# noc-lab/sac-expert

Measured on NVIDIA B200. Metric: agent-updates/sec, higher is better.
Workload: dtype f32

## Files before the change

sac_expert_b200/csrc/mlp_ws.cuh:

```cuda
#pragma once
#include "tc_gemm.cuh"
#include "planes.cuh"

namespace saceo {

constexpr int WS_NEW = 16;
constexpr int WS_NEPI = WS_NEW * 32, WS_NT = WS_NEPI + 64;
constexpr int WS_NST = 3, WS_RING = WS_NST * WS_STAGE;
constexpr int WS_AUX = 49152;
constexpr int WS_PATCH1 = 32 * 32 * 4;
constexpr int WS_PATCH = WS_NEW * WS_PATCH1;
constexpr int WS_MAIN = WS_RING + WS_AUX + WS_PATCH;
constexpr int WS_BYTES = WS_MAIN + 1024 + 256;
constexpr int WS_RED = 40960;
constexpr int WS_MAXOUT = 36;
enum { WB_FULL = 0, WB_EMPTY = WS_NST, WB_XFULL = 2 * WS_NST, WB_XEMPTY, WB_D0, WB_D1, WB_AP , WB_D2 = WB_AP + 4 };

__device__ __forceinline__ void mbar_arrive(uint32_t bar) {
  asm volatile("mbarrier.arrive.shared::cta.b64 _, [%0];" ::"r"(bar) : "memory");
}
__device__ __forceinline__ void mbar_expect_tx(uint32_t bar, uint32_t bytes) {
  asm volatile("mbarrier.arrive.expect_tx.shared::cta.b64 _, [%0], %1;" ::"r"(bar), "r"(bytes) : "memory");
}
__device__ __forceinline__ void bulk_g2s(uint32_t dst, const void* src, uint32_t bytes, uint32_t bar) {
  asm volatile("cp.async.bulk.shared::cluster.global.mbarrier::complete_tx::bytes [%0], [%1], %2, [%3];"
               ::"r"(dst), "l"(src), "r"(bytes), "r"(bar) : "memory");
}
__device__ __forceinline__ void bulk_prefetch_l2(const void* src, uint32_t bytes) {
  asm volatile("cp.async.bulk.prefetch.L2.global [%0], %1;" ::"l"(src), "r"(bytes) : "memory");
}
__device__ __forceinline__ void epi_bar() { asm volatile("bar.sync 1, 512;" ::: "memory"); }
__device__ __forceinline__ uint64_t umma_desc_mn(uint32_t saddr, uint32_t lbo = 4096) {
  return (uint64_t)((saddr >> 4) & 0x3FFF) | ((uint64_t)(lbo >> 4) << 16) | ((uint64_t)(1024 >> 4) << 32) |
         ((uint64_t)1 << 46) | ((uint64_t)2 << 61);
}
constexpr uint32_t WS_IDESC_FWD = (1u << 4) | (1u << 16) | ((uint32_t)(256 >> 3) << 17) | ((uint32_t)(128 >> 4) << 24);
constexpr uint32_t WS_IDESC_BWD = (1u << 4) | ((uint32_t)(128 >> 3) << 17) | ((uint32_t)(128 >> 4) << 24);

__global__ void k_planes_build(const float* __restrict__ theta, long long stride, uint8_t* __restrict__ img, int K0, int nout) {
  const int n0 = (K0 + 31) / 32, N2 = ws_w2_rows(nout), rows = n0 * 32 + 256 + N2;
  const int item = blockIdx.x * blockDim.x + threadIdx.x;
  if (item >= rows * 32) return;
  const int row = item >> 5, c8 = item & 31;
  const float* th = theta + (long long)blockIdx.y * stride;
  uint8_t* net_img = img + (long long)blockIdx.y * ws_image_bytes(K0, nout);
  float x[8];
  if (row >= n0 * 32 + 256) {
    const int n = row - n0 * 32 - 256;
    const long long o = (long long)K0 * 256 + 256 + 65536 + 256 + (long long)(c8 * 8) * nout + n;
#pragma unroll
    for (int j = 0; j < 8; ++j) x[j] = n < nout ? th[o + (long long)j * nout] * WS_W2_SCALE : 0.f;
    uint4 hi, lo;
    split8<true>(x, hi, lo);
    uint8_t* dst = net_img + (long long)(n0 + 8) * WS_STAGE + ws_w2_off(N2, n, c8);
    *reinterpret_cast<uint4*>(dst) = hi;
    *reinterpret_cast<uint4*>(dst + N2 * 128) = lo;
    return;
  }
  if (row < n0 * 32) {
#pragma unroll
    for (int j = 0; j < 8; ++j) x[j] = row < K0 ? th[(long long)row * 256 + c8 * 8 + j] : 0.f;
  } else {
    const long long o = (long long)K0 * 256 + 256 + (long long)(row - n0 * 32) * 256 + c8 * 8;
#pragma unroll
    for (int j = 0; j < 8; ++j) x[j] = th[o + j];
  }
  uint4 hi, lo;
  split8<true>(x, hi, lo);
  uint8_t* dst = net_img + ws_image_off(row, c8);
  *reinterpret_cast<uint4*>(dst) = hi;
  *reinterpret_cast<uint4*>(dst + 16384) = lo;
}

__device__ __forceinline__ uint32_t ws_pa(uint32_t patch, int r, int c) {
  return patch + (uint32_t)(r * 128 + ((((c >> 2) ^ (r & 7)) << 4) | ((c & 3) << 2)));
}
__device__ __forceinline__ void ws_store_rows(uint32_t patch, const uint32_t (&v)[32], float* __restrict__ G, int rbase,
                                              int rows, int col, int lane, uint32_t cs = 0, int q = 0) {
#pragma unroll
  for (int j = 0; j < 8; ++j) sts128(ws_pa(patch, lane, 4 * j), make_uint4(v[4 * j], v[4 * j + 1], v[4 * j + 2], v[4 * j + 3]));
  __syncwarp();
  const int lr = lane >> 3, lc = (lane & 7) * 4;
  float4 sum = make_float4(0.f, 0.f, 0.f, 0.f);
#pragma unroll
  for (int rr = 0; rr < 32; rr += 4) {
    const int r = rr + lr, grow = rbase + r;
    if (grow < rows) {
      const float4 t4 = lds128(ws_pa(patch, r, lc));
      if (G) *reinterpret_cast<float4*>(G + (long long)grow * FW_H + col + lc) = t4;
      sum.x += t4.x; sum.y += t4.y; sum.z += t4.z; sum.w += t4.w;
    }
  }
  if (cs) {
#pragma unroll
    for (int o = 8; o <= 16; o <<= 1) {
      sum.x += __shfl_xor_sync(0xffffffffu, sum.x, o); sum.y += __shfl_xor_sync(0xffffffffu, sum.y, o);
      sum.z += __shfl_xor_sync(0xffffffffu, sum.z, o); sum.w += __shfl_xor_sync(0xffffffffu, sum.w, o);
    }
    if (lane < 8) sts128f(cs + (uint32_t)(q * FW_H + col + lc) * 4, sum.x, sum.y, sum.z, sum.w);
// ... 170 lines not shown
__device__ __forceinline__ void ws_split_store(uint32_t taddr, const uint32_t (&v)[32], float scale) {
#pragma unroll
  for (int h = 0; h < 2; ++h) {
    uint32_t hi[8], lo[8];
#pragma unroll
    for (int j = 0; j < 8; ++j) {
      const float x0 = __uint_as_float(v[16 * h + 2 * j]) * scale, x1 = __uint_as_float(v[16 * h + 2 * j + 1]) * scale;
      asm("cvt.rn.satfinite.f16x2.f32 %0, %1, %2;" : "=r"(hi[j]) : "f"(x1), "f"(x0));
      const float2 hf = __half22float2(*reinterpret_cast<const __half2*>(&hi[j]));
      asm("cvt.rn.satfinite.f16x2.f32 %0, %1, %2;" : "=r"(lo[j]) : "f"(x1 - hf.y), "f"(x0 - hf.x));
    }
    tmem_st8(taddr + 8 * h, hi);
    tmem_st8(taddr + 16 + 8 * h, lo);
  }
}
template <int ACT>
__device__ __forceinline__ void ws_mul_dact_p(uint32_t (&v)[32], uint32_t patch, int lane, float s) {
#pragma unroll
  for (int j = 0; j < 8; ++j) {
    const float4 h = lds128(ws_pa(patch, lane, 4 * j));
    v[4 * j] = __float_as_uint(__uint_as_float(v[4 * j]) * s * dact_from_out(ACT, h.x));
    v[4 * j + 1] = __float_as_uint(__uint_as_float(v[4 * j + 1]) * s * dact_from_out(ACT, h.y));
    v[4 * j + 2] = __float_as_uint(__uint_as_float(v[4 * j + 2]) * s * dact_from_out(ACT, h.z));
    v[4 * j + 3] = __float_as_uint(__uint_as_float(v[4 * j + 3]) * s * dact_from_out(ACT, h.w));
  }
  __syncwarp();
}
__device__ __forceinline__ void ws_mul_dact_p_rt(int act, uint32_t (&v)[32], uint32_t patch, int lane, float s) {
  if (act == ACT_RELU) ws_mul_dact_p<ACT_RELU>(v, patch, lane, s);
  else if (act == ACT_TANH) ws_mul_dact_p<ACT_TANH>(v, patch, lane, s);
  else ws_mul_dact_p<ACT_ELU>(v, patch, lane, s);
}
__device__ __forceinline__ void ws_rows_commit_p(uint32_t patch, int lane, const float4 (&t)[8]) {
  const int lr = lane >> 3, lc = (lane & 7) * 4;
#pragma unroll
  for (int i = 0; i < 8; ++i)
    sts128(ws_pa(patch, 4 * i + lr, lc), make_uint4(__float_as_uint(t[i].x), __float_as_uint(t[i].y), __float_as_uint(t[i].z), __float_as_uint(t[i].w)));
  __syncwarp();
}
__device__ __forceinline__ void ws_split_f16(const uint32_t (&v)[32], float scale, uint32_t (&hi)[16], uint32_t (&lo)[16]) {
#pragma unroll
  for (int j = 0; j < 16; ++j) {
    const float x0 = __uint_as_float(v[2 * j]) * scale, x1 = __uint_as_float(v[2 * j + 1]) * scale;
    asm("cvt.rn.satfinite.f16x2.f32 %0, %1, %2;" : "=r"(hi[j]) : "f"(x1), "f"(x0));
    const float2 hf = __half22float2(*reinterpret_cast<const __half2*>(&hi[j]));
    asm("cvt.rn.satfinite.f16x2.f32 %0, %1, %2;" : "=r"(lo[j]) : "f"(x1 - hf.y), "f"(x0 - hf.x));
  }
}
template <int ACT>
__device__ __forceinline__ void ws_bias_act(uint32_t (&v)[32], uint32_t bias) {
#pragma unroll
  for (int j = 0; j < 8; ++j) {
    const float4 b = lds128(bias + j * 16);
    v[4 * j] = __float_as_uint(apply_act(ACT, __uint_as_float(v[4 * j]) + b.x));
    v[4 * j + 1] = __float_as_uint(apply_act(ACT, __uint_as_float(v[4 * j + 1]) + b.y));
    v[4 * j + 2] = __float_as_uint(apply_act(ACT, __uint_as_float(v[4 * j + 2]) + b.z));
    v[4 * j + 3] = __float_as_uint(apply_act(ACT, __uint_as_float(v[4 * j + 3]) + b.w));
  }
}
__device__ __forceinline__ void ws_bias_act_rt(int act, uint32_t (&v)[32], uint32_t bias) {
  if (act == ACT_RELU) ws_bias_act<ACT_RELU>(v, bias);
  else if (act == ACT_TANH) ws_bias_act<ACT_TANH>(v, bias);
  else ws_bias_act<ACT_ELU>(v, bias);
}
template <int ACT>
__device__ __forceinline__ void ws_mul_dact(uint32_t (&v)[32], const float (&aux)[32], float s) {
#pragma unroll
  for (int j = 0; j < 32; ++j) v[j] = __float_as_uint(__uint_as_float(v[j]) * s * dact_from_out(ACT, aux[j]));
}
__device__ __forceinline__ void ws_mul_dact_rt(int act, uint32_t (&v)[32], const float (&aux)[32], float s) {
  if (act == ACT_RELU) ws_mul_dact<ACT_RELU>(v, aux, s);
  else if (act == ACT_TANH) ws_mul_dact<ACT_TANH>(v, aux, s);
  else ws_mul_dact<ACT_ELU>(v, aux, s);
}
__device__ __forceinline__ float ws_row_scale(float bound) {
  if (!(bound > 0.f) || !(bound < 3.0e38f)) return 1.f;
  int e;
  frexpf(bound, &e);
  e = 10 - e;
  e = e > 120 ? 120 : (e < -120 ? -120 : e);
  return ldexpf(1.f, e);
}

struct FwdW {
  const float* X; int ldx; long long sXa, sXn;
  const float* theta; long long sTa, sTn;
  const uint8_t* planes; long long sPa, sPn;
  float* H1; float* H2; long long sHa, sHn;
  uint8_t* H1p; long long sQa, sQn;
  float* Out; int ldo; long long sOa, sOn;
  int rows, K0, nout, nnet, act0, act1;
  unsigned long long* dbg;
};
#define WS_STAMP(i) do { if (f.dbg && lane == 0) f.dbg[(size_t)(blockIdx.y * gridDim.x + blockIdx.x) * 16 + (i)] = gtime(); } while (0)

__global__ void __launch_bounds__(WS_NT, 1) k_mlp_fwd_ws(FwdW f) {
  extern __shared__ uint8_t smem_raw[];
  const uint32_t sb = (smem_u32(smem_raw) + 1023u) & ~1023u;
  const uint32_t ring = sb, aux = sb + WS_RING, patch_base = aux + WS_AUX, bars = sb + WS_MAIN, tslot = bars + 8 * 16;
  auto bar = [&](int i) { return bars + 8u * (uint32_t)i; };
  const int z = blockIdx.y, agent = z / f.nnet, net = z - agent * f.nnet;
  const int row0 = blockIdx.x * TC_BM;
  const int warp = threadIdx.x >> 5, lane = threadIdx.x & 31;
  const int n0 = (f.K0 + 31) >> 5, nk64 = (f.K0 + 63) >> 6;
  const int N2 = ws_w2_rows(f.nout);
  const uint32_t idesc_out = (1u << 4) | ((uint32_t)(N2 >> 3) << 17) | ((uint32_t)(128 >> 4) << 24);

  if (threadIdx.x == 0) {
    for (int s = 0; s < 2 * WS_NST; ++s) mbar_init(bar(s), 1);
    mbar_init(bar(WB_XFULL), WS_NEW); mbar_init(bar(WB_XEMPTY), 1);
    mbar_init(bar(WB_D0), 1); mbar_init(bar(WB_D1), 1); mbar_init(bar(WB_D2), 1);
    for (int g = 0; g < 4; ++g) mbar_init(bar(WB_AP + g), 8);
    asm volatile("fence.mbarrier_init.release.cluster;" ::: "memory");
  }
  if (warp == WS_NEW + 1) {
    asm volatile("tcgen05.alloc.cta_group::1.sync.aligned.shared::cta.b32 [%0], %1;" ::"r"(tslot), "n"(512) : "memory");
    asm volatile("tcgen05.relinquish_alloc_permit.cta_group::1.sync.aligned;" ::: "memory");
  }
  asm volatile("tcgen05.fence::before_thread_sync;" ::: "memory");
  __syncthreads();
  asm volatile("tcgen05.fence::after_thread_sync;" ::: "memory");
  const uint32_t tmem = lds_u32(tslot);
  const uint32_t tP = tmem, tQ = tmem + 256;

  if (warp == WS_NEW) {
    if (lane == 0) {
      const uint8_t* img = f.planes + agent * f.sPa + net * f.sPn;
      const int total = n0 + 8 + (N2 ? 2 : 0);
      const uint32_t w2_item = (uint32_t)N2 * 512;
      auto item_src = [&](int it) { return it < n0 + 8 ? img + (long long)it * WS_STAGE : img + (long long)(n0 + 8) * WS_STAGE + (it - n0 - 8) * w2_item; };
      for (int it = 0; it < total; ++it) {
        const int s = it % WS_NST;
        const uint32_t bytes = it < n0 + 8 ? (uint32_t)WS_STAGE : w2_item;
        mbar_wait(bar(WB_EMPTY + s), (uint32_t)(((it / WS_NST) & 1) ^ 1));
        mbar_expect_tx(bar(WB_FULL + s), bytes);
        bulk_g2s(ring + s * WS_STAGE, item_src(it), bytes, bar(WB_FULL + s));
        if (it == WS_NST - 1)
          for (int j = WS_NST; j < total; ++j) bulk_prefetch_l2(item_src(j), j < n0 + 8 ? (uint32_t)WS_STAGE : w2_item);
      }
      WS_STAMP(11);
    }
  } else if (warp == WS_NEW + 1) {
    if (lane == 0) {
      int it = 0;
      for (int sl = 0; sl < nk64; ++sl) {
        mbar_wait(bar(WB_XFULL), (uint32_t)(sl & 1));
        asm volatile("tcgen05.fence::after_thread_sync;" ::: "memory");
        for (int hh = 0; hh < 2 && sl * 2 + hh < n0; ++hh, ++it) {
          const int s = it % WS_NST;
          mbar_wait(bar(WB_FULL + s), (uint32_t)((it / WS_NST) & 1));
          asm volatile("tcgen05.fence::after_thread_sync;" ::: "memory");
          const uint32_t st = ring + s * WS_STAGE;
#pragma unroll
          for (int kk = 0; kk < 2; ++kk) {
            const uint32_t ka = (uint32_t)(hh * 2 + kk) * 32, kb = (uint32_t)kk * 2048;
            umma_f16(tP, umma_desc(aux + ka), umma_desc_mn(st + kb), WS_IDESC_FWD, (it | kk) ? 1u : 0u);
            umma_f16(tP, umma_desc(aux + ka), umma_desc_mn(st + 16384 + kb), WS_IDESC_FWD, 1u);
            umma_f16(tP, umma_desc(aux + 16384 + ka), umma_desc_mn(st + kb), WS_IDESC_FWD, 1u);
          }
          umma_commit(bar(WB_EMPTY + s));
        }
        umma_commit(bar(WB_XEMPTY));
      }
      umma_commit(bar(WB_D0));
      WS_STAMP(8);
      for (int g = 0; g < 4; ++g) {
        mbar_wait(bar(WB_AP + g), 0);
        asm volatile("tcgen05.fence::after_thread_sync;" ::: "memory");
        if (g == 3) WS_STAMP(9);
        for (int tt = 0; tt < 2; ++tt, ++it) {
          const int t = 2 * g + tt, s = it % WS_NST;
          mbar_wait(bar(WB_FULL + s), (uint32_t)((it / WS_NST) & 1));
          asm volatile("tcgen05.fence::after_thread_sync;" ::: "memory");
          const uint32_t st = ring + s * WS_STAGE;
#pragma unroll
          for (int kk = 0; kk < 2; ++kk) {
            const uint32_t ta_hi = tP + 32 * t + 8 * kk, ta_lo = ta_hi + 16, kb = (uint32_t)kk * 2048;
            umma_f16_ts(tQ, ta_hi, umma_desc_mn(st + kb), WS_IDESC_FWD, (t | kk) ? 1u : 0u);
            umma_f16_ts(tQ, ta_hi, umma_desc_mn(st + 16384 + kb), WS_IDESC_FWD, 1u);
            umma_f16_ts(tQ, ta_lo, umma_desc_mn(st + kb), WS_IDESC_FWD, 1u);
          }
          umma_commit(bar(WB_EMPTY + s));
        }
      }
      umma_commit(bar(WB_D1));
      WS_STAMP(10);
      if (N2) {
        for (int w = 0; w < 2; ++w, ++it) {
          const int s = it % WS_NST;
          mbar_wait(bar(WB_FULL + s), (uint32_t)((it / WS_NST) & 1));
          asm volatile("tcgen05.fence::after_thread_sync;" ::: "memory");
          for (int gg = 0; gg < 2; ++gg) {
            const int g = 2 * w + gg;
            mbar_wait(bar(WB_AP + g), 1);
            asm volatile("tcgen05.fence::after_thread_sync;" ::: "memory");
            const uint32_t bh = ring + s * WS_STAGE + (uint32_t)(gg * N2 * 256), bl = bh + (uint32_t)N2 * 128;
#pragma unroll
            for (int kk = 0; kk < 4; ++kk) {
              const uint32_t ta_hi = tQ + 64 * g + 32 * (kk >> 1) + 8 * (kk & 1), ta_lo = ta_hi + 16, kb = (uint32_t)kk * 32;
              umma_f16_ts(tP, ta_hi, umma_desc(bh + kb), idesc_out, (g | kk) ? 1u : 0u);
              umma_f16_ts(tP, ta_hi, umma_desc(bl + kb), idesc_out, 1u);
              umma_f16_ts(tP, ta_lo, umma_desc(bh + kb), idesc_out, 1u);
            }
          }
          umma_commit(bar(WB_EMPTY + s));
        }
        umma_commit(bar(WB_D2));
      }
    }
  } else {
    const int q = warp & 3, cg = warp >> 2;
    const uint32_t lane_addr = (uint32_t)(q * 32) << 16;
    const uint32_t patch = patch_base + (uint32_t)warp * WS_PATCH1;
    const int rbase = row0 + q * 32, grow = rbase + lane;
    const float* __restrict__ X = f.X + agent * f.sXa + net * f.sXn;
    const float* __restrict__ th = f.theta + agent * f.sTa + net * f.sTn;
    const long long ob0 = (long long)f.K0 * FW_H, oW1 = ob0 + FW_H, ob1 = oW1 + (long long)FW_H * FW_H,
                    oW2 = ob1 + FW_H, ob2 = oW2 + (long long)FW_H * f.nout;
    float* H1 = f.H1 ? f.H1 + agent * f.sHa + net * f.sHn : nullptr;
    float* H2 = f.H2 ? f.H2 + agent * f.sHa + net * f.sHn : nullptr;
    float* Out = f.Out + agent * f.sOa + net * f.sOn;
    if (warp == 0) WS_STAMP(0);
    const uint32_t cb0 = aux + WS_RED + 2048, cb1 = cb0 + 1024, cw2 = cb1 + 1024, cb2 = cw2 + 1024;
    if (threadIdx.x < FW_H) {
      const int t = threadIdx.x;
      asm volatile("st.shared.f32 [%0], %1;" ::"r"(cb0 + t * 4), "f"(__ldg(th + ob0 + t)) : "memory");
      asm volatile("st.shared.f32 [%0], %1;" ::"r"(cb1 + t * 4), "f"(__ldg(th + ob1 + t)) : "memory");
      if (f.nout == 1) asm volatile("st.shared.f32 [%0], %1;" ::"r"(cw2 + t * 4), "f"(__ldg(th + oW2 + t)) : "memory");
      if (t < f.nout) asm volatile("st.shared.f32 [%0], %1;" ::"r"(cb2 + t * 4), "f"(__ldg(th + ob2 + t)) : "memory");
    }
    {
      Slab<TC_BM, WS_NEPI> sx;
      sx.init(X, f.ldx, 1, row0, f.rows);
      for (int sl = 0; sl < nk64; ++sl) {
        sx.ld(sl * 64, f.K0);
        if (sl > 0) mbar_wait(bar(WB_XEMPTY), (uint32_t)((sl - 1) & 1));
        sx.template st<true>(aux, aux + 16384);
        asm volatile("fence.proxy.async.shared::cta;" ::: "memory");
        __syncwarp();
        if (lane == 0) mbar_arrive(bar(WB_XFULL));
      }
    }
    epi_bar();
    if (warp == 0) WS_STAMP(1);
    mbar_wait(bar(WB_D0), 0);
    asm volatile("tcgen05.fence::after_thread_sync;" ::: "memory");
    if (warp == 0) WS_STAMP(2);
#pragma unroll 1
    for (int c = 0; c < 2; ++c) {
      const int kg = 2 * c + (cg >> 1), col = kg * 64 + (cg & 1) * 32;
      uint32_t v[32];
      tmem_ld32(tP + lane_addr + (uint32_t)col, v);
      ws_bias_act_rt(f.act0, v, cb0 + col * 4);
      ws_split_store(tP + lane_addr + (uint32_t)col, v, 1.f);
      {
        asm volatile("tcgen05.wait::st.sync.aligned;" ::: "memory");
        asm volatile("tcgen05.fence::before_thread_sync;" ::: "memory");
        __syncwarp();
        if (lane == 0) mbar_arrive(bar(WB_AP + kg));
      }
      if (f.H1p) {
#pragma unroll
        for (int j = 0; j < 8; ++j) sts128(ws_pa(patch, lane, 4 * j), make_uint4(v[4 * j], v[4 * j + 1], v[4 * j + 2], v[4 * j + 3]));
        __syncwarp();
        ws_store_planes_p(patch, f.H1p + agent * f.sQa + net * f.sQn, rbase, f.rows, col, lane);
        __syncwarp();
      } else if (H1) { ws_store_rows(patch, v, H1, rbase, f.rows, col, lane); __syncwarp(); }
    }
    if (warp == 0) WS_STAMP(3);
    if (warp == 0) WS_STAMP(4);
    mbar_wait(bar(WB_D1), 0);
    asm volatile("tcgen05.fence::after_thread_sync;" ::: "memory");
    if (warp == 0) WS_STAMP(5);
    if (N2) {
#pragma unroll 1
      for (int c = 0; c < 2; ++c) {
        const int kg = 2 * c + (cg >> 1), col = kg * 64 + (cg & 1) * 32;
        uint32_t v[32];
        tmem_ld32(tQ + lane_addr + (uint32_t)col, v);
        ws_bias_act_rt(f.act1, v, cb1 + col * 4);
        ws_split_store(tQ + lane_addr + (uint32_t)col, v, 1.f);
        {
          asm volatile("tcgen05.wait::st.sync.aligned;" ::: "memory");
          asm volatile("tcgen05.fence::before_thread_sync;" ::: "memory");
          __syncwarp();
          if (lane == 0) mbar_arrive(bar(WB_AP + kg));
        }
        if (H2) { ws_store_rows(patch, v, H2, rbase, f.rows, col, lane); __syncwarp(); }
      }
      if (warp == 0) WS_STAMP(6);
      if (cg == 0) {
        mbar_wait(bar(WB_D2), 0);
        asm volatile("tcgen05.fence::after_thread_sync;" ::: "memory");
        for (int r0 = 0; r0 < N2; r0 += 32) {
          uint32_t v[32];
          tmem_ld32(tP + lane_addr + (uint32_t)r0, v);
          if (grow < f.rows) {
#pragma unroll
            for (int cc = 0; cc < 32; ++cc)
              if (r0 + cc < f.nout) Out[(long long)grow * f.ldo + r0 + cc] = __uint_as_float(v[cc]) * (1.f / WS_W2_SCALE) + lds32(cb2 + (uint32_t)(r0 + cc) * 4);
          }
        }
      }
    } else {
      float qacc = 0.f;
#pragma unroll 1
      for (int c = 0; c < 2; ++c) {
        const int col = cg * 64 + c * 32;
        uint32_t v[32];
        tmem_ld32(tQ + lane_addr + (uint32_t)col, v);
        ws_bias_act_rt(f.act1, v, cb1 + col * 4);
        if (H2) { ws_store_rows(patch, v, H2, rbase, f.rows, col, lane); __syncwarp(); }
#pragma unroll
        for (int j = 0; j < 8; ++j) {
          const float4 t4 = lds128(cw2 + (uint32_t)(col + 4 * j) * 4);
          qacc = fmaf(__uint_as_float(v[4 * j]), t4.x, qacc); qacc = fmaf(__uint_as_float(v[4 * j + 1]), t4.y, qacc);
          qacc = fmaf(__uint_as_float(v[4 * j + 2]), t4.z, qacc); qacc = fmaf(__uint_as_float(v[4 * j + 3]), t4.w, qacc);
        }
      }
      if (warp == 0) WS_STAMP(6);
      const uint32_t red = aux + WS_RED;
      if (cg > 0) asm volatile("st.shared.f32 [%0], %1;" ::"r"(red + (uint32_t)((cg - 1) * TC_BM + q * 32 + lane) * 4), "f"(qacc) : "memory");
      epi_bar();
      if (cg == 0 && grow < f.rows) {
        const uint32_t r = red + (uint32_t)(q * 32 + lane) * 4;
        Out[(long long)grow * f.ldo] = ((qacc + lds32(r)) + (lds32(r + TC_BM * 4) + lds32(r + 2 * TC_BM * 4))) + lds32(cb2);
      }
    }
    if (warp == 0) WS_STAMP(7);
  }
  asm volatile("tcgen05.fence::before_thread_sync;" ::: "memory");
  __syncthreads();
  if (warp == WS_NEW + 1) {
    asm volatile("tcgen05.dealloc.cta_group::1.sync.aligned.b32 %0, %1;" ::"r"(tmem), "n"(512) : "memory");
  }
}

struct BwdW {
  const float* dOut; int ldd; long long sDa, sDn; int kout;
  const float* theta; long long sTa, sTn; int K0, nout;
  const uint8_t* planes; long long sPa, sPn;
  const float* H1; const float* H2; long long sHa, sHn;
  float* dH2; float* dH1;
  uint8_t* dH2p; long long sQa, sQn;
  uint8_t* dH1p;
  const uint8_t* H1p;
  float* dXa; int s_cols, a_cols; long long sXa, sXn;
  int rows, nnet, act0, act1;
  float* dbpart;
  unsigned long long* dbg;
};

template <int NG, int NA, int MODE>
__global__ void __launch_bounds__(WS_NT, 1) k_mlp_bwd_ws(BwdW f) {
  extern __shared__ uint8_t smem_raw[];
  const uint32_t sb = (smem_u32(smem_raw) + 1023u) & ~1023u;
  const uint32_t ring = sb, aux = sb + WS_RING, patch_base = aux + WS_AUX, bars = sb + WS_MAIN, tslot = bars + 8 * 16;
  const uint32_t cs2 = aux + WS_RED, cs1 = cs2 + 4096;
  auto bar = [&](int i) { return bars + 8u * (uint32_t)i; };
  const int z = blockIdx.y, agent = z / f.nnet, net = z - agent * f.nnet;
  const int row0 = blockIdx.x * TC_BM;
  const int warp = threadIdx.x >> 5, lane = threadIdx.x & 31;
  const int n0 = (f.K0 + 31) >> 5;

  if (threadIdx.x == 0) {
    for (int s = 0; s < 2 * WS_NST; ++s) mbar_init(bar(s), 1);
    mbar_init(bar(WB_D0), 1); mbar_init(bar(WB_D1), 1);
    for (int g = 0; g < 4; ++g) mbar_init(bar(WB_AP + g), 8);
    mbar_init(bar(WB_XFULL), 4); mbar_init(bar(WB_XEMPTY), 1);
    asm volatile("fence.mbarrier_init.release.cluster;" ::: "memory");
    asm volatile("st.shared.u32 [%0], %1;" ::"r"(aux + WS_RED - 256), "r"(0u) : "memory");
  }
  if (warp == WS_NEW + 1) {
    asm volatile("tcgen05.alloc.cta_group::1.sync.aligned.shared::cta.b32 [%0], %1;" ::"r"(tslot), "n"(512) : "memory");
    asm volatile("tcgen05.relinquish_alloc_permit.cta_group::1.sync.aligned;" ::: "memory");
  }
  asm volatile("tcgen05.fence::before_thread_sync;" ::: "memory");
  __syncthreads();
  asm volatile("tcgen05.fence::after_thread_sync;" ::: "memory");
  const uint32_t tmem = lds_u32(tslot);
  const uint32_t tP = tmem, tQ = tmem + 256;

  if (warp == WS_NEW) {
    if (lane == 0) {
      const uint8_t* w1 = f.planes + agent * f.sPa + net * f.sPn + (long long)n0 * WS_STAGE;
      if (NG > 0) {
        const int N2 = ws_w2_rows(f.nout);
        const uint8_t* w2 = w1 + 8LL * WS_STAGE;
        for (int pl = 0; pl < 2; ++pl) {
          mbar_expect_tx(bar(WB_FULL + pl), (uint32_t)N2 * 512);
          for (int sj = 0; sj < 4; ++sj)
            bulk_g2s(ring + pl * WS_STAGE + sj * N2 * 128, w2 + (sj * 2 + pl) * N2 * 128, (uint32_t)N2 * 128, bar(WB_FULL + pl));
        }
      }
      for (int i = 0; i < 8; ++i) {
        const int it = i + (NG > 0 ? 2 : 0), h = i >> 2, sj = i & 3, s = it % WS_NST;
        mbar_wait(bar(WB_EMPTY + s), (uint32_t)(((it / WS_NST) & 1) ^ 1));
        mbar_expect_tx(bar(WB_FULL + s), WS_STAGE);
        for (int pl = 0; pl < 2; ++pl)
          for (int tt = 0; tt < 4; ++tt)
            bulk_g2s(ring + s * WS_STAGE + pl * 16384 + tt * 4096,
                     w1 + (long long)(4 * h + tt) * WS_STAGE + pl * 16384 + sj * 4096, 4096, bar(WB_FULL + s));
        if (it == WS_NST - 1)
          for (int t = 0; t < 8; ++t) bulk_prefetch_l2(w1 + (long long)t * WS_STAGE, WS_STAGE);
      }
    }
  } else if (warp == WS_NEW + 1) {
    if (lane == 0) {
      if (NG > 0) {
        const uint32_t lbo = (uint32_t)ws_w2_rows(f.nout) * 128;
        mbar_wait(bar(WB_XFULL), 0);
        mbar_wait(bar(WB_FULL + 0), 0);
// ... 403 lines not shown
        for (int j = 0; j < 8; ++j) x8[j] = 8 * c8 + j < f.in ? v8[j] : 0.f;
      }
      uint4 hi, lo;
      split8<false>(x8, hi, lo);
      const uint32_t dst = xs + (uint32_t)t * DW0_XST + (uint32_t)r * 128 + (uint32_t)((c8 ^ (r & 7)) << 4);
      sts128(dst, hi); sts128(dst + 4096, lo);
    }
    asm volatile("fence.proxy.async.shared::cta;" ::: "memory");
    epi_bar();
    if (threadIdx.x == 0) mbar_arrive(bar(2 * DW0_NST + 1));
  }
  if (warp == WS_NEW + 1) {
    if (lane == 0) {
      mbar_wait(bar(2 * DW0_NST + 1), 0);
      asm volatile("tcgen05.fence::after_thread_sync;" ::: "memory");
      for (int it = 0; it < nst; ++it) {
        const int s = it % DW0_NST;
        mbar_wait(bar(s), (uint32_t)((it / DW0_NST) & 1));
        asm volatile("tcgen05.fence::after_thread_sync;" ::: "memory");
        const uint32_t sa = xs + (uint32_t)it * DW0_XST, sbb = ring + s * WS_STAGE;
#pragma unroll
        for (int kk = 0; kk < 2; ++kk) {
          const uint32_t ko = (uint32_t)kk * 2048;
          const uint32_t a_hi = sa + ko, a_lo = a_hi + 4096, b_hi = sbb + ko, b_lo = b_hi + 16384, acc = (it | kk) ? 1u : 0u;
          umma_f16(tmem, umma_desc_mn(a_hi), umma_desc_mn(b_hi), DW_IDESC, acc);
          umma_f16(tmem, umma_desc_mn(a_hi), umma_desc_mn(b_lo), DW_IDESC, 1u);
          umma_f16(tmem, umma_desc_mn(a_lo), umma_desc_mn(b_hi), DW_IDESC, 1u);
        }
        umma_commit(bar(DW0_NST + s));
      }
      umma_commit(bar(2 * DW0_NST));
    }
  } else if (warp < WS_NEW) {
    const int q = warp & 3, cg = warp >> 2;
    if (q * 32 < f.in) {
      const uint32_t lane_addr = (uint32_t)(q * 32) << 16;
      const uint32_t patch = ring + (uint32_t)warp * WS_PATCH1;
      float* G = f.G + agent * f.sGa + net * f.sGn;
      mbar_wait(bar(2 * DW0_NST), 0);
      asm volatile("tcgen05.fence::after_thread_sync;" ::: "memory");
#pragma unroll 1
      for (int c = 0; c < 2; ++c) {
        const int col = cg * 64 + c * 32;
        uint32_t v[32];
        tmem_ld32(tmem + lane_addr + (uint32_t)col, v);
        ws_store_rows(patch, v, G, q * 32, f.in, col, lane);
        __syncwarp();
      }
    }
  }
  asm volatile("tcgen05.fence::before_thread_sync;" ::: "memory");
  __syncthreads();
  if (warp == WS_NEW + 1) {
    asm volatile("tcgen05.dealloc.cta_group::1.sync.aligned.b32 %0, %1;" ::"r"(tmem), "n"(256) : "memory");
  }
}
static inline bool dw0_planes_eligible(int in, int rows, int ldx, const float* X, long long sXa, long long sXn) {
  return in >= 1 && in <= 64 && ((rows + 31) >> 5) <= DW0_MAXST && (ldx % 4) == 0 && (reinterpret_cast<uintptr_t>(X) & 15) == 0 &&
         (sXa % 4) == 0 && (sXn % 4) == 0;
}

static inline cudaError_t mlp_ws_init() {
  static bool done_dev[64] = {};
  int dev_ = 0; cudaGetDevice(&dev_);
  bool& done = done_dev[dev_ & 63];
  if (done) return cudaSuccess;
  cudaError_t e;
#define WS_ATTR(K) e = cudaFuncSetAttribute(K, cudaFuncAttributeMaxDynamicSharedMemorySize, WS_BYTES); if (e) return e;
  WS_ATTR(k_mlp_fwd_ws)
  WS_ATTR((k_mlp_bwd_ws<0, 0, 0>)) WS_ATTR((k_mlp_bwd_ws<0, 1, 0>)) WS_ATTR((k_mlp_bwd_ws<0, 2, 0>))
  WS_ATTR((k_mlp_bwd_ws<1, 0, 0>)) WS_ATTR((k_mlp_bwd_ws<2, 0, 0>)) WS_ATTR((k_mlp_bwd_ws<3, 0, 0>))
  WS_ATTR((k_mlp_bwd_ws<0, 0, 1>)) WS_ATTR((k_mlp_bwd_ws<1, 0, 1>)) WS_ATTR((k_mlp_bwd_ws<0, 1, 2>))
#undef WS_ATTR
  e = cudaFuncSetAttribute(k_dw_planes, cudaFuncAttributeMaxDynamicSharedMemorySize, DW_BYTES); if (e) return e;
  e = cudaFuncSetAttribute(k_dw0_planes, cudaFuncAttributeMaxDynamicSharedMemorySize, DW0_BYTES); if (e) return e;
  done = true;
  return cudaSuccess;
}
static inline bool mlp_fwd_ws_eligible(int h1, int h2, int nout, int K0, const float* theta, long long sTa, long long sTn) {
  return h1 == FW_H && h2 == FW_H && nout >= 1 && nout <= WS_MAXOUT && K0 >= 1 &&
         ((reinterpret_cast<uintptr_t>(theta) & 15) == 0) && ((sTa & 3) == 0) && ((sTn & 3) == 0);
}
static inline cudaError_t mlp_fwd_ws_launch(const FwdW& f, int nagents, cudaStream_t st) {
  dim3 grid((f.rows + TC_BM - 1) / TC_BM, nagents * f.nnet);
  k_mlp_fwd_ws<<<grid, WS_NT, WS_BYTES, st>>>(f);
  return cudaPeekAtLastError();
}
static inline bool mlp_bwd_ws_eligible(int h1, int h2, int kout, int nout, bool want_dxa, int a_cols, const float* theta, long long sTa,
                                       long long sTn) {
  if (!(h1 == FW_H && h2 == FW_H && kout >= 1 && kout <= WS_MAXOUT && kout <= nout)) return false;
  if (want_dxa && (kout != 1 || a_cols < 1 || a_cols > 32)) return false;
  return ((reinterpret_cast<uintptr_t>(theta) & 15) == 0) && ((sTa & 3) == 0) && ((sTn & 3) == 0);
}
static inline cudaError_t mlp_bwd_ws_launch(const BwdW& f, int nagents, cudaStream_t st) {
  dim3 grid((f.rows + TC_BM - 1) / TC_BM, nagents * f.nnet);
  const int ng = f.kout == 1 ? 0 : (f.kout + 15) / 16, na = f.dXa ? (f.a_cols + 15) / 16 : 0;
  const bool m1 = f.H1p && f.dH2p && f.dH1p && !f.dH2 && !f.dH1, m2 = f.H1p && !f.dH2p && !f.dH1p && !f.dH2 && !f.dH1;
  if (ng == 0 && na == 0 && m1) k_mlp_bwd_ws<0, 0, 1><<<grid, WS_NT, WS_BYTES, st>>>(f);
  else if (ng == 1 && na == 0 && m1) k_mlp_bwd_ws<1, 0, 1><<<grid, WS_NT, WS_BYTES, st>>>(f);
  else if (ng == 0 && na == 1 && m2) k_mlp_bwd_ws<0, 1, 2><<<grid, WS_NT, WS_BYTES, st>>>(f);
  else if (ng == 0 && na == 0) k_mlp_bwd_ws<0, 0, 0><<<grid, WS_NT, WS_BYTES, st>>>(f);
  else if (ng == 0 && na == 1) k_mlp_bwd_ws<0, 1, 0><<<grid, WS_NT, WS_BYTES, st>>>(f);
  else if (ng == 0) k_mlp_bwd_ws<0, 2, 0><<<grid, WS_NT, WS_BYTES, st>>>(f);
  else if (ng == 1) k_mlp_bwd_ws<1, 0, 0><<<grid, WS_NT, WS_BYTES, st>>>(f);
  else if (ng == 2) k_mlp_bwd_ws<2, 0, 0><<<grid, WS_NT, WS_BYTES, st>>>(f);
  else k_mlp_bwd_ws<3, 0, 0><<<grid, WS_NT, WS_BYTES, st>>>(f);
  return cudaPeekAtLastError();
}

}
```

Measured before the change: 132,900.

## Chain four row tiles per CTA in the forward warp-specialized MLP kernel

The forward kernel becomes semi-persistent: each CTA processes up to four consecutive (agent, net, row-tile) tiles instead of one. This amortizes TMEM allocation, barrier setup and launch cost across tiles. It also overlaps the next tile's constant staging and first X-slab conversion with the current tile's second layer, using double-buffered constant slots and a new D2R barrier so TMEM is not reused before it has been read. The cost is fewer CTAs, which can underfill the SMs when the tile count is small, plus more intricate phase bookkeeping and a risk of ordering bugs.

New measurement: 127,600, median of 6. 0.96x the previous value.

```diff
diff --git a/sac_expert_b200/csrc/mlp_ws.cuh b/sac_expert_b200/csrc/mlp_ws.cuh
--- a/sac_expert_b200/csrc/mlp_ws.cuh
+++ b/sac_expert_b200/csrc/mlp_ws.cuh
@@ -14,7 +14,7 @@
 constexpr int WS_BYTES = WS_MAIN + 1024 + 256;
 constexpr int WS_RED = 40960;
 constexpr int WS_MAXOUT = 36;
-enum { WB_FULL = 0, WB_EMPTY = WS_NST, WB_XFULL = 2 * WS_NST, WB_XEMPTY, WB_D0, WB_D1, WB_AP , WB_D2 = WB_AP + 4 };
+enum { WB_FULL = 0, WB_EMPTY = WS_NST, WB_XFULL = 2 * WS_NST, WB_XEMPTY, WB_D0, WB_D1, WB_AP , WB_D2 = WB_AP + 4, WB_D2R };
 
 __device__ __forceinline__ void mbar_arrive(uint32_t bar) {
   asm volatile("mbarrier.arrive.shared::cta.b64 _, [%0];" ::"r"(bar) : "memory");
@@ -351,6 +351,8 @@
   return ldexpf(1.f, e);
 }
 
+constexpr int WS_CHAIN = 4;
+constexpr int WS_CONST1 = 32768;
 struct FwdW {
   const float* X; int ldx; long long sXa, sXn;
   const float* theta; long long sTa, sTn;
@@ -362,14 +364,15 @@
   unsigned long long* dbg;
 };
 #define WS_STAMP(i) do { if (f.dbg && lane == 0) f.dbg[(size_t)(blockIdx.y * gridDim.x + blockIdx.x) * 16 + (i)] = gtime(); } while (0)
-
-__global__ void __launch_bounds__(WS_NT, 1) k_mlp_fwd_ws(FwdW f) {
+#define WS_TSTAMP(i) do { if (f.dbg && lane == 0) f.dbg[(size_t)T * 16 + (i)] = gtime(); } while (0)
+
+__global__ void __launch_bounds__(WS_NT, 1) k_mlp_fwd_ws(FwdW f, int ntiles) {
   extern __shared__ uint8_t smem_raw[];
   const uint32_t sb = (smem_u32(smem_raw) + 1023u) & ~1023u;
   const uint32_t ring = sb, aux = sb + WS_RING, patch_base = aux + WS_AUX, bars = sb + WS_MAIN, tslot = bars + 8 * 16;
   auto bar = [&](int i) { return bars + 8u * (uint32_t)i; };
-  const int z = blockIdx.y, agent = z / f.nnet, net = z - agent * f.nnet;
-  const int row0 = blockIdx.x * TC_BM;
+  const int nrt = (f.rows + TC_BM - 1) / TC_BM;
+  const int T0 = blockIdx.x * WS_CHAIN, nt = min(WS_CHAIN, ntiles - T0);
   const int warp = threadIdx.x >> 5, lane = threadIdx.x & 31;
   const int n0 = (f.K0 + 31) >> 5, nk64 = (f.K0 + 63) >> 6;
   const int N2 = ws_w2_rows(f.nout);
@@ -380,6 +383,7 @@
     mbar_init(bar(WB_XFULL), WS_NEW); mbar_init(bar(WB_XEMPTY), 1);
     mbar_init(bar(WB_D0), 1); mbar_init(bar(WB_D1), 1); mbar_init(bar(WB_D2), 1);
     for (int g = 0; g < 4; ++g) mbar_init(bar(WB_AP + g), 8);
+    mbar_init(bar(WB_D2R), 4);
     asm volatile("fence.mbarrier_init.release.cluster;" ::: "memory");
   }
   if (warp == WS_NEW + 1) {
@@ -394,209 +398,259 @@
 
   if (warp == WS_NEW) {
     if (lane == 0) {
-      const uint8_t* img = f.planes + agent * f.sPa + net * f.sPn;
-      const int total = n0 + 8 + (N2 ? 2 : 0);
+      const int per = n0 + 8 + (N2 ? 2 : 0);
       const uint32_t w2_item = (uint32_t)N2 * 512;
-      auto item_src = [&](int it) { return it < n0 + 8 ? img + (long long)it * WS_STAGE : img + (long long)(n0 + 8) * WS_STAGE + (it - n0 - 8) * w2_item; };
-      for (int it = 0; it < total; ++it) {
-        const int s = it % WS_NST;
-        const uint32_t bytes = it < n0 + 8 ? (uint32_t)WS_STAGE : w2_item;
-        mbar_wait(bar(WB_EMPTY + s), (uint32_t)(((it / WS_NST) & 1) ^ 1));
-        mbar_expect_tx(bar(WB_FULL + s), bytes);
-        bulk_g2s(ring + s * WS_STAGE, item_src(it), bytes, bar(WB_FULL + s));
-        if (it == WS_NST - 1)
-          for (int j = WS_NST; j < total; ++j) bulk_prefetch_l2(item_src(j), j < n0 + 8 ? (uint32_t)WS_STAGE : w2_item);
-      }
-      WS_STAMP(11);
+      auto img_of = [&](int T) {
+        const int z = T / nrt, agent = z / f.nnet;
+        return f.planes + agent * f.sPa + (z - agent * f.nnet) * f.sPn;
+      };
+      auto item_src = [&](const uint8_t* img, int k) {
+        return k < n0 + 8 ? img + (long long)k * WS_STAGE : img + (long long)(n0 + 8) * WS_STAGE + (k - n0 - 8) * w2_item;
+      };
+      auto item_bytes = [&](int k) { return k < n0 + 8 ? (uint32_t)WS_STAGE : w2_item; };
+      int it = 0;
+      for (int j = 0; j < nt; ++j) {
+        const int T = T0 + j;
+        const uint8_t* img = img_of(T);
+        for (int k = 0; k < per; ++k, ++it) {
+          const int s = it % WS_NST;
+          mbar_wait(bar(WB_EMPTY + s), (uint32_t)(((it / WS_NST) & 1) ^ 1));
+          mbar_expect_tx(bar(WB_FULL + s), item_bytes(k));
+          bulk_g2s(ring + s * WS_STAGE, item_src(img, k), item_bytes(k), bar(WB_FULL + s));
+          if (k == WS_NST - 1) {
+            if (j == 0)
+              for (int kk = WS_NST; kk < per; ++kk) bulk_prefetch_l2(item_src(img, kk), item_bytes(kk));
+            if (j + 1 < nt && (T + 1) / nrt != T / nrt) {
+              const uint8_t* nimg = img_of(T + 1);
+              for (int kk = 0; kk < per; ++kk) bulk_prefetch_l2(item_src(nimg, kk), item_bytes(kk));
+            }
+          }
+        }
+        WS_TSTAMP(11);
+      }
     }
   } else if (warp == WS_NEW + 1) {
     if (lane == 0) {
       int it = 0;
-      for (int sl = 0; sl < nk64; ++sl) {
-        mbar_wait(bar(WB_XFULL), (uint32_t)(sl & 1));
-        asm volatile("tcgen05.fence::after_thread_sync;" ::: "memory");
-        for (int hh = 0; hh < 2 && sl * 2 + hh < n0; ++hh, ++it) {
-          const int s = it % WS_NST;
-          mbar_wait(bar(WB_FULL + s), (uint32_t)((it / WS_NST) & 1));
+      for (int j = 0; j < nt; ++j) {
+        const int T = T0 + j;
+        const uint32_t ph = (uint32_t)j & 1u, ap = (uint32_t)(j * (N2 ? 2 : 1));
+        if (j > 0) {
+          mbar_wait(bar(N2 ? WB_D2R : WB_D1), ph ^ 1u);
           asm volatile("tcgen05.fence::after_thread_sync;" ::: "memory");
-          const uint32_t st = ring + s * WS_STAGE;
-#pragma unroll
-          for (int kk = 0; kk < 2; ++kk) {
-            const uint32_t ka = (uint32_t)(hh * 2 + kk) * 32, kb = (uint32_t)kk * 2048;
-            umma_f16(tP, umma_desc(aux + ka), umma_desc_mn(st + kb), WS_IDESC_FWD, (it | kk) ? 1u : 0u);
-            umma_f16(tP, umma_desc(aux + ka), umma_desc_mn(st + 16384 + kb), WS_IDESC_FWD, 1u);
-            umma_f16(tP, umma_desc(aux + 16384 + ka), umma_desc_mn(st + kb), WS_IDESC_FWD, 1u);
+        }
+        const int it0 = it;
+        for (int sl = 0; sl < nk64; ++sl) {
+          mbar_wait(bar(WB_XFULL), (uint32_t)((j * nk64 + sl) & 1));
+          asm volatile("tcgen05.fence::after_thread_sync;" ::: "memory");
+          for (int hh = 0; hh < 2 && sl * 2 + hh < n0; ++hh, ++it) {
+            const int s = it % WS_NST;
+            mbar_wait(bar(WB_FULL + s), (uint32_t)((it / WS_NST) & 1));
+            asm volatile("tcgen05.fence::after_thread_sync;" ::: "memory");
+            const uint32_t st = ring + s * WS_STAGE;
+#pragma unroll
+            for (int kk = 0; kk < 2; ++kk) {
+              const uint32_t ka = (uint32_t)(hh * 2 + kk) * 32, kb = (uint32_t)kk * 2048;
+              umma_f16(tP, umma_desc(aux + ka), umma_desc_mn(st + kb), WS_IDESC_FWD, ((it - it0) | kk) ? 1u : 0u);
+              umma_f16(tP, umma_desc(aux + ka), umma_desc_mn(st + 16384 + kb), WS_IDESC_FWD, 1u);
+              umma_f16(tP, umma_desc(aux + 16384 + ka), umma_desc_mn(st + kb), WS_IDESC_FWD, 1u);
+            }
+            umma_commit(bar(WB_EMPTY + s));
           }
-          umma_commit(bar(WB_EMPTY + s));
-        }
-        umma_commit(bar(WB_XEMPTY));
-      }
-      umma_commit(bar(WB_D0));
-      WS_STAMP(8);
-      for (int g = 0; g < 4; ++g) {
-        mbar_wait(bar(WB_AP + g), 0);
-        asm volatile("tcgen05.fence::after_thread_sync;" ::: "memory");
-        if (g == 3) WS_STAMP(9);
-        for (int tt = 0; tt < 2; ++tt, ++it) {
-          const int t = 2 * g + tt, s = it % WS_NST;
-          mbar_wait(bar(WB_FULL + s), (uint32_t)((it / WS_NST) & 1));
+          umma_commit(bar(WB_XEMPTY));
+        }
+        umma_commit(bar(WB_D0));
+        WS_TSTAMP(8);
+        for (int g = 0; g < 4; ++g) {
+          mbar_wait(bar(WB_AP + g), ap & 1u);
           asm volatile("tcgen05.fence::after_thread_sync;" ::: "memory");
-          const uint32_t st = ring + s * WS_STAGE;
-#pragma unroll
-          for (int kk = 0; kk < 2; ++kk) {
-            const uint32_t ta_hi = tP + 32 * t + 8 * kk, ta_lo = ta_hi + 16, kb = (uint32_t)kk * 2048;
-            umma_f16_ts(tQ, ta_hi, umma_desc_mn(st + kb), WS_IDESC_FWD, (t | kk) ? 1u : 0u);
-            umma_f16_ts(tQ, ta_hi, umma_desc_mn(st + 16384 + kb), WS_IDESC_FWD, 1u);
-            umma_f16_ts(tQ, ta_lo, umma_desc_mn(st + kb), WS_IDESC_FWD, 1u);
+          if (g == 3) WS_TSTAMP(9);
+          for (int tt = 0; tt < 2; ++tt, ++it) {
+            const int t = 2 * g + tt, s = it % WS_NST;
+            mbar_wait(bar(WB_FULL + s), (uint32_t)((it / WS_NST) & 1));
+            asm volatile("tcgen05.fence::after_thread_sync;" ::: "memory");
+            const uint32_t st = ring + s * WS_STAGE;
+#pragma unroll
+            for (int kk = 0; kk < 2; ++kk) {
+              const uint32_t ta_hi = tP + 32 * t + 8 * kk, ta_lo = ta_hi + 16, kb = (uint32_t)kk * 2048;
+              umma_f16_ts(tQ, ta_hi, umma_desc_mn(st + kb), WS_IDESC_FWD, (t | kk) ? 1u : 0u);
+              umma_f16_ts(tQ, ta_hi, umma_desc_mn(st + 16384 + kb), WS_IDESC_FWD, 1u);
+              umma_f16_ts(tQ, ta_lo, umma_desc_mn(st + kb), WS_IDESC_FWD, 1u);
+            }
+            umma_commit(bar(WB_EMPTY + s));
           }
-          umma_commit(bar(WB_EMPTY + s));
-        }
-      }
-      umma_commit(bar(WB_D1));
-      WS_STAMP(10);
-      if (N2) {
-        for (int w = 0; w < 2; ++w, ++it) {
-          const int s = it % WS_NST;
-          mbar_wait(bar(WB_FULL + s), (uint32_t)((it / WS_NST) & 1));
-          asm volatile("tcgen05.fence::after_thread_sync;" ::: "memory");
-          for (int gg = 0; gg < 2; ++gg) {
-            const int g = 2 * w + gg;
-            mbar_wait(bar(WB_AP + g), 1);
+        }
+        umma_commit(bar(WB_D1));
+        WS_TSTAMP(10);
+        if (N2) {
+          for (int w = 0; w < 2; ++w, ++it) {
+            const int s = it % WS_NST;
+            mbar_wait(bar(WB_FULL + s), (uint32_t)((it / WS_NST) & 1));
             asm volatile("tcgen05.fence::after_thread_sync;" ::: "memory");
-            const uint32_t bh = ring + s * WS_STAGE + (uint32_t)(gg * N2 * 256), bl = bh + (uint32_t)N2 * 128;
-#pragma unroll
-            for (int kk = 0; kk < 4; ++kk) {
-              const uint32_t ta_hi = tQ + 64 * g + 32 * (kk >> 1) + 8 * (kk & 1), ta_lo = ta_hi + 16, kb = (uint32_t)kk * 32;
-              umma_f16_ts(tP, ta_hi, umma_desc(bh + kb), idesc_out, (g | kk) ? 1u : 0u);
-              umma_f16_ts(tP, ta_hi, umma_desc(bl + kb), idesc_out, 1u);
-              umma_f16_ts(tP, ta_lo, umma_desc(bh + kb), idesc_out, 1u);
+            for (int gg = 0; gg < 2; ++gg) {
+              const int g = 2 * w + gg;
+              mbar_wait(bar(WB_AP + g), (ap + 1u) & 1u);
+              asm volatile("tcgen05.fence::after_thread_sync;" ::: "memory");
+              const uint32_t bh = ring + s * WS_STAGE + (uint32_t)(gg * N2 * 256), bl = bh + (uint32_t)N2 * 128;
+#pragma unroll
+              for (int kk = 0; kk < 4; ++kk) {
+                const uint32_t ta_hi = tQ + 64 * g + 32 * (kk >> 1) + 8 * (kk & 1), ta_lo = ta_hi + 16, kb = (uint32_t)kk * 32;
+                umma_f16_ts(tP, ta_hi, umma_desc(bh + kb), idesc_out, (g | kk) ? 1u : 0u);
+                umma_f16_ts(tP, ta_hi, umma_desc(bl + kb), idesc_out, 1u);
+                umma_f16_ts(tP, ta_lo, umma_desc(bh + kb), idesc_out, 1u);
+              }
             }
+            umma_commit(bar(WB_EMPTY + s));
           }
-          umma_commit(bar(WB_EMPTY + s));
-        }
-        umma_commit(bar(WB_D2));
+          umma_commit(bar(WB_D2));
+        }
       }
     }
   } else {
     const int q = warp & 3, cg = warp >> 2;
     const uint32_t lane_addr = (uint32_t)(q * 32) << 16;
     const uint32_t patch = patch_base + (uint32_t)warp * WS_PATCH1;
-    const int rbase = row0 + q * 32, grow = rbase + lane;
-    const float* __restrict__ X = f.X + agent * f.sXa + net * f.sXn;
-    const float* __restrict__ th = f.theta + agent * f.sTa + net * f.sTn;
-    const long long ob0 = (long long)f.K0 * FW_H, oW1 = ob0 + FW_H, ob1 = oW1 + (long long)FW_H * FW_H,
-                    oW2 = ob1 + FW_H, ob2 = oW2 + (long long)FW_H * f.nout;
-    float* H1 = f.H1 ? f.H1 + agent * f.sHa + net * f.sHn : nullptr;
-    float* H2 = f.H2 ? f.H2 + agent * f.sHa + net * f.sHn : nullptr;
-    float* Out = f.Out + agent * f.sOa + net * f.sOn;
-    if (warp == 0) WS_STAMP(0);
-    const uint32_t cb0 = aux + WS_RED + 2048, cb1 = cb0 + 1024, cw2 = cb1 + 1024, cb2 = cw2 + 1024;
-    if (threadIdx.x < FW_H) {
-      const int t = threadIdx.x;
-      asm volatile("st.shared.f32 [%0], %1;" ::"r"(cb0 + t * 4), "f"(__ldg(th + ob0 + t)) : "memory");
-      asm volatile("st.shared.f32 [%0], %1;" ::"r"(cb1 + t * 4), "f"(__ldg(th + ob1 + t)) : "memory");
-      if (f.nout == 1) asm volatile("st.shared.f32 [%0], %1;" ::"r"(cw2 + t * 4), "f"(__ldg(th + oW2 + t)) : "memory");
-      if (t < f.nout) asm volatile("st.shared.f32 [%0], %1;" ::"r"(cb2 + t * 4), "f"(__ldg(th + ob2 + t)) : "memory");
-    }
-    {
+    auto consts_of = [&](int j) { return (j & 1) ? aux + WS_CONST1 : aux + WS_RED + 2048; };
+    auto stage_consts = [&](int T, uint32_t cb0) {
+      if (threadIdx.x < FW_H) {
+        const int z = T / nrt, agent = z / f.nnet, t = threadIdx.x;
+        const float* __restrict__ th = f.theta + agent * f.sTa + (z - agent * f.nnet) * f.sTn;
+        const long long ob0 = (long long)f.K0 * FW_H, ob1 = ob0 + FW_H + (long long)FW_H * FW_H, oW2 = ob1 + FW_H,
+                        ob2 = oW2 + (long long)FW_H * f.nout;
+        asm volatile("st.shared.f32 [%0], %1;" ::"r"(cb0 + t * 4), "f"(__ldg(th + ob0 + t)) : "memory");
+        asm volatile("st.shared.f32 [%0], %1;" ::"r"(cb0 + 1024 + t * 4), "f"(__ldg(th + ob1 + t)) : "memory");
+        if (f.nout == 1) asm volatile("st.shared.f32 [%0], %1;" ::"r"(cb0 + 2048 + t * 4), "f"(__ldg(th + oW2 + t)) : "memory");
+        if (t < f.nout) asm volatile("st.shared.f32 [%0], %1;" ::"r"(cb0 + 3072 + t * 4), "f"(__ldg(th + ob2 + t)) : "memory");
+      }
+    };
+    auto convert_x = [&](int T, int s0, int s1, int xs) {
+      const int z = T / nrt, agent = z / f.nnet;
       Slab<TC_BM, WS_NEPI> sx;
-      sx.init(X, f.ldx, 1, row0, f.rows);
-      for (int sl = 0; sl < nk64; ++sl) {
+      sx.init(f.X + agent * f.sXa + (z - agent * f.nnet) * f.sXn, f.ldx, 1, (T - z * nrt) * TC_BM, f.rows);
+      for (int sl = s0; sl < s1; ++sl, ++xs) {
         sx.ld(sl * 64, f.K0);
-        if (sl > 0) mbar_wait(bar(WB_XEMPTY), (uint32_t)((sl - 1) & 1));
+        if (xs > 0) mbar_wait(bar(WB_XEMPTY), (uint32_t)((xs - 1) & 1));
         sx.template st<true>(aux, aux + 16384);
         asm volatile("fence.proxy.async.shared::cta;" ::: "memory");
         __syncwarp();
         if (lane == 0) mbar_arrive(bar(WB_XFULL));
       }
-    }
-    epi_bar();
-    if (warp == 0) WS_STAMP(1);
-    mbar_wait(bar(WB_D0), 0);
-    asm volatile("tcgen05.fence::after_thread_sync;" ::: "memory");
-    if (warp == 0) WS_STAMP(2);
+    };
 #pragma unroll 1
-    for (int c = 0; c < 2; ++c) {
-      const int kg = 2 * c + (cg >> 1), col = kg * 64 + (cg & 1) * 32;
-      uint32_t v[32];
-      tmem_ld32(tP + lane_addr + (uint32_t)col, v);
-      ws_bias_act_rt(f.act0, v, cb0 + col * 4);
-      ws_split_store(tP + lane_addr + (uint32_t)col, v, 1.f);
-      {
-        asm volatile("tcgen05.wait::st.sync.aligned;" ::: "memory");
-        asm volatile("tcgen05.fence::before_thread_sync;" ::: "memory");
-        __syncwarp();
-        if (lane == 0) mbar_arrive(bar(WB_AP + kg));
-      }
-      if (f.H1p) {
-#pragma unroll
-        for (int j = 0; j < 8; ++j) sts128(ws_pa(patch, lane, 4 * j), make_uint4(v[4 * j], v[4 * j + 1], v[4 * j + 2], v[4 * j + 3]));
-        __syncwarp();
-        ws_store_planes_p(patch, f.H1p + agent * f.sQa + net * f.sQn, rbase, f.rows, col, lane);
-        __syncwarp();
-      } else if (H1) { ws_store_rows(patch, v, H1, rbase, f.rows, col, lane); __syncwarp(); }
-    }
-    if (warp == 0) WS_STAMP(3);
-    if (warp == 0) WS_STAMP(4);
-    mbar_wait(bar(WB_D1), 0);
-    asm volatile("tcgen05.fence::after_thread_sync;" ::: "memory");
-    if (warp == 0) WS_STAMP(5);
-    if (N2) {
+    for (int j = 0; j < nt; ++j) {
+      const int T = T0 + j;
+      const int rbase = (T % nrt) * TC_BM + q * 32, grow = rbase + lane;
+      auto off = [&](long long sa, long long sn) {
+        int t;
+        asm volatile("mov.b32 %0, %1;" : "=r"(t) : "r"(T));
+        const int z = t / nrt, agent = z / f.nnet;
+        return agent * sa + (z - agent * f.nnet) * sn;
+      };
+      const uint32_t ph = (uint32_t)j & 1u;
+      const uint32_t cb0 = consts_of(j), cb1 = cb0 + 1024, cw2 = cb1 + 1024, cb2 = cw2 + 1024;
+      if (warp == 0) WS_TSTAMP(0);
+      if (j == 0) {
+        stage_consts(T, cb0);
+        convert_x(T, 0, nk64, 0);
+      } else if (nk64 > 1) {
+        convert_x(T, 1, nk64, j * nk64 + 1);
+      }
+      asm volatile("tcgen05.fence::before_thread_sync;" ::: "memory");
+      epi_bar();
+      if (warp == 0) WS_TSTAMP(1);
+      mbar_wait(bar(WB_D0), ph);
+      asm volatile("tcgen05.fence::after_thread_sync;" ::: "memory");
+      if (warp == 0) WS_TSTAMP(2);
 #pragma unroll 1
       for (int c = 0; c < 2; ++c) {
         const int kg = 2 * c + (cg >> 1), col = kg * 64 + (cg & 1) * 32;
         uint32_t v[32];
-        tmem_ld32(tQ + lane_addr + (uint32_t)col, v);
-        ws_bias_act_rt(f.act1, v, cb1 + col * 4);
-        ws_split_store(tQ + lane_addr + (uint32_t)col, v, 1.f);
+        tmem_ld32(tP + lane_addr + (uint32_t)col, v);
+        ws_bias_act_rt(f.act0, v, cb0 + col * 4);
+        ws_split_store(tP + lane_addr + (uint32_t)col, v, 1.f);
         {
           asm volatile("tcgen05.wait::st.sync.aligned;" ::: "memory");
           asm volatile("tcgen05.fence::before_thread_sync;" ::: "memory");
           __syncwarp();
           if (lane == 0) mbar_arrive(bar(WB_AP + kg));
         }
-        if (H2) { ws_store_rows(patch, v, H2, rbase, f.rows, col, lane); __syncwarp(); }
-      }
-      if (warp == 0) WS_STAMP(6);
-      if (cg == 0) {
-        mbar_wait(bar(WB_D2), 0);
-        asm volatile("tcgen05.fence::after_thread_sync;" ::: "memory");
-        for (int r0 = 0; r0 < N2; r0 += 32) {
+        if (f.H1p) {
+#pragma unroll
+          for (int jj = 0; jj < 8; ++jj) sts128(ws_pa(patch, lane, 4 * jj), make_uint4(v[4 * jj], v[4 * jj + 1], v[4 * jj + 2], v[4 * jj + 3]));
+          __syncwarp();
+          ws_store_planes_p(patch, f.H1p + off(f.sQa, f.sQn), rbase, f.rows, col, lane);
+          __syncwarp();
+        } else if (f.H1) { ws_store_rows(patch, v, f.H1 + off(f.sHa, f.sHn), rbase, f.rows, col, lane); __syncwarp(); }
+      }
+      if (warp == 0) WS_TSTAMP(3);
+      if (j + 1 < nt) {
+        stage_consts(T + 1, consts_of(j + 1));
+        convert_x(T + 1, 0, 1, (j + 1) * nk64);
+      }
+      if (warp == 0) WS_TSTAMP(4);
+      mbar_wait(bar(WB_D1), ph);
+      asm volatile("tcgen05.fence::after_thread_sync;" ::: "memory");
+      if (warp == 0) WS_TSTAMP(5);
+      if (N2) {
+#pragma unroll 1
+        for (int c = 0; c < 2; ++c) {
+          const int kg = 2 * c + (cg >> 1), col = kg * 64 + (cg & 1) * 32;
           uint32_t v[32];
-          tmem_ld32(tP + lane_addr + (uint32_t)r0, v);
-          if (grow < f.rows) {
-#pragma unroll
-            for (int cc = 0; cc < 32; ++cc)
-              if (r0 + cc < f.nout) Out[(long long)grow * f.ldo + r0 + cc] = __uint_as_float(v[cc]) * (1.f / WS_W2_SCALE) + lds32(cb2 + (uint32_t)(r0 + cc) * 4);
+          tmem_ld32(tQ + lane_addr + (uint32_t)col, v);
+          ws_bias_act_rt(f.act1, v, cb1 + col * 4);
+          ws_split_store(tQ + lane_addr + (uint32_t)col, v, 1.f);
+          {
+            asm volatile("tcgen05.wait::st.sync.aligned;" ::: "memory");
+            asm volatile("tcgen05.fence::before_thread_sync;" ::: "memory");
+            __syncwarp();
+            if (lane == 0) mbar_arrive(bar(WB_AP + kg));
           }
-        }
-      }
-    } else {
-      float qacc = 0.f;
+          if (f.H2) { ws_store_rows(patch, v, f.H2 + off(f.sHa, f.sHn), rbase, f.rows, col, lane); __syncwarp(); }
+        }
+        if (warp == 0) WS_TSTAMP(6);
+        if (cg == 0) {
+          mbar_wait(bar(WB_D2), ph);
+          asm volatile("tcgen05.fence::after_thread_sync;" ::: "memory");
+          for (int r0 = 0; r0 < N2; r0 += 32) {
+            uint32_t v[32];
+            tmem_ld32(tP + lane_addr + (uint32_t)r0, v);
+            if (grow < f.rows) {
+#pragma unroll
+              for (int cc = 0; cc < 32; ++cc)
+                if (r0 + cc < f.nout) f.Out[off(f.sOa, f.sOn) + (long long)grow * f.ldo + r0 + cc] = __uint_as_float(v[cc]) * (1.f / WS_W2_SCALE) + lds32(cb2 + (uint32_t)(r0 + cc) * 4);
+            }
+          }
+          asm volatile("tcgen05.fence::before_thread_sync;" ::: "memory");
+          __syncwarp();
+          if (lane == 0) mbar_arrive(bar(WB_D2R));
+        }
+      } else {
+        float qacc = 0.f;
 #pragma unroll 1
-      for (int c = 0; c < 2; ++c) {
-        const int col = cg * 64 + c * 32;
-        uint32_t v[32];
-        tmem_ld32(tQ + lane_addr + (uint32_t)col, v);
-        ws_bias_act_rt(f.act1, v, cb1 + col * 4);
-        if (H2) { ws_store_rows(patch, v, H2, rbase, f.rows, col, lane); __syncwarp(); }
-#pragma unroll
-        for (int j = 0; j < 8; ++j) {
-          const float4 t4 = lds128(cw2 + (uint32_t)(col + 4 * j) * 4);
-          qacc = fmaf(__uint_as_float(v[4 * j]), t4.x, qacc); qacc = fmaf(__uint_as_float(v[4 * j + 1]), t4.y, qacc);
-          qacc = fmaf(__uint_as_float(v[4 * j + 2]), t4.z, qacc); qacc = fmaf(__uint_as_float(v[4 * j + 3]), t4.w, qacc);
-        }
-      }
-      if (warp == 0) WS_STAMP(6);
-      const uint32_t red = aux + WS_RED;
-      if (cg > 0) asm volatile("st.shared.f32 [%0], %1;" ::"r"(red + (uint32_t)((cg - 1) * TC_BM + q * 32 + lane) * 4), "f"(qacc) : "memory");
-      epi_bar();
-      if (cg == 0 && grow < f.rows) {
-        const uint32_t r = red + (uint32_t)(q * 32 + lane) * 4;
-        Out[(long long)grow * f.ldo] = ((qacc + lds32(r)) + (lds32(r + TC_BM * 4) + lds32(r + 2 * TC_BM * 4))) + lds32(cb2);
-      }
-    }
-    if (warp == 0) WS_STAMP(7);
+        for (int c = 0; c < 2; ++c) {
+          const int col = cg * 64 + c * 32;
+          uint32_t v[32];
+          tmem_ld32(tQ + lane_addr + (uint32_t)col, v);
+          ws_bias_act_rt(f.act1, v, cb1 + col * 4);
+          if (f.H2) { ws_store_rows(patch, v, f.H2 + off(f.sHa, f.sHn), rbase, f.rows, col, lane); __syncwarp(); }
+#pragma unroll
+          for (int jj = 0; jj < 8; ++jj) {
+            const float4 t4 = lds128(cw2 + (uint32_t)(col + 4 * jj) * 4);
+            qacc = fmaf(__uint_as_float(v[4 * jj]), t4.x, qacc); qacc = fmaf(__uint_as_float(v[4 * jj + 1]), t4.y, qacc);
+            qacc = fmaf(__uint_as_float(v[4 * jj + 2]), t4.z, qacc); qacc = fmaf(__uint_as_float(v[4 * jj + 3]), t4.w, qacc);
+          }
+        }
+        if (warp == 0) WS_TSTAMP(6);
+        const uint32_t red = aux + WS_RED;
+        if (cg > 0) asm volatile("st.shared.f32 [%0], %1;" ::"r"(red + (uint32_t)((cg - 1) * TC_BM + q * 32 + lane) * 4), "f"(qacc) : "memory");
+        epi_bar();
+        if (cg == 0 && grow < f.rows) {
+          const uint32_t r = red + (uint32_t)(q * 32 + lane) * 4;
+          f.Out[off(f.sOa, f.sOn) + (long long)grow * f.ldo] = ((qacc + lds32(r)) + (lds32(r + TC_BM * 4) + lds32(r + 2 * TC_BM * 4))) + lds32(cb2);
+        }
+      }
+      if (warp == 0) WS_TSTAMP(7);
+    }
   }
   asm volatile("tcgen05.fence::before_thread_sync;" ::: "memory");
   __syncthreads();
@@ -1166,8 +1220,8 @@
          ((reinterpret_cast<uintptr_t>(theta) & 15) == 0) && ((sTa & 3) == 0) && ((sTn & 3) == 0);
 }
 static inline cudaError_t mlp_fwd_ws_launch(const FwdW& f, int nagents, cudaStream_t st) {
-  dim3 grid((f.rows + TC_BM - 1) / TC_BM, nagents * f.nnet);
-  k_mlp_fwd_ws<<<grid, WS_NT, WS_BYTES, st>>>(f);
+  const int tiles = (f.rows + TC_BM - 1) / TC_BM * nagents * f.nnet;
+  k_mlp_fwd_ws<<<(tiles + WS_CHAIN - 1) / WS_CHAIN, WS_NT, WS_BYTES, st>>>(f, tiles);
   return cudaPeekAtLastError();
 }
 static inline bool mlp_bwd_ws_eligible(int h1, int h2, int kout, int nout, bool want_dxa, int a_cols, const float* theta, long long sTa,
```
